# davnords/octic-vits

Measured on AMD Instinct MI355X. Metric: images/sec Hybrid Octic ViT-H/14 224² bf16 train step @1/2/4/8 MI355X, higher is better.
Workload: dtype bf16; 1 GPU; hybrid_deit_huge_patch14 (16 octic + 16 standard blocks, drop_path 0.5) DeiT-III train step: bf16-autocast fwd + bwd + LAMB + EMA, 224x224, batch 64/GPU (BASELINE configs[1]), data parallel over 1 GPU(s); global_batch=64, per_gpu_batch=64, accum_steps=1, parallelism=dp1, library_gemm_table=True, launch=hipGraph replay (whole step)

## Files before the change

include/octic_hip.h:

```cpp
#ifndef OCTIC_HIP_H
#define OCTIC_HIP_H

#include <stdint.h>

#ifdef __cplusplus
extern "C" {
#endif

#define OCTIC_ABI_VERSION 20

enum { OCTIC_F32 = 0, OCTIC_BF16 = 1, OCTIC_U8 = 2  };

enum {
  OCTIC_OK = 0,
  OCTIC_ESHAPE = -1,
  OCTIC_EALIGN = -2,
  OCTIC_EDTYPE = -3,
  OCTIC_ENULL = -4,
  OCTIC_EWORKSPACE = -5
};

typedef struct {
  void* ptr[5];
  int64_t ld[5];
// ... 3 lines not shown
const char* octic_strerror(int code);

enum {
  OCTIC_ROUTE_DENSE_TILE = 0,
  OCTIC_ROUTE_DENSE_SPLIT = 1,
  OCTIC_ROUTE_WGRAD_SLABS = 2,
  OCTIC_ROUTE_WGRAD_TILE = 3,
  OCTIC_ROUTE_LINEAR_RING = 4,
  OCTIC_ROUTE_RING_EVEN = 5,
  OCTIC_ROUTE_ATTN_LEGACY = 6,
  OCTIC_ROUTE_ATTN_ONLINE = 7,
  OCTIC_ROUTE_ATTN_BWD_PAIR = 8,
  OCTIC_ROUTE_DENSE_IMAGE = 9,
  OCTIC_ROUTE_DENSE_CLS2 = 10,
  OCTIC_ROUTE_ATTN_STREAM = 11,
  OCTIC_ROUTE_COUNT = 12
};
int octic_route_override(int knob, int value);

int octic_gelu_d8_fwd(const octic_view* x, const octic_view* y, int64_t M, int c, int dtype, void* stream);
int octic_gelu_d8_bwd(const octic_view* g, const octic_view* x, const octic_view* gin, int64_t M, int c,
                      int dtype, void* stream);
int octic_gelu_d8_fwd_skip(const octic_view* x, const octic_view* y, int64_t M, int c, int dtype,
                           const float* sample_scale, int64_t rows_per_sample, void* stream);
int octic_gelu_d8_bwd_skip(const octic_view* g, const octic_view* x, const octic_view* gin, int64_t M, int c, int dtype,
                           const float* sample_scale, int64_t rows_per_sample, void* stream);

int octic_layernorm_d8_fwd(const octic_view* x, const octic_view* y, const float* const alpha[5],
                           const float* beta, float* stats, int64_t M, int c, float eps, int out_dtype,
                           void* stream);
int octic_layernorm_d8_bwd_blocks(int64_t M);
// ... 66 lines not shown
int octic_linear_d8_ring_order_dropped(int ngroups, const int* items, const int* ksteps, int slots_per_xcd, const int* n_chunks,
                                       const unsigned char* dead_long, const unsigned char* dead_short, int* out_group,
                                       int* out_item, int* out_dead);

int octic_linear_d8_wgrad_has_colsum(int cin, int cout, int dtype);
enum {
  OCTIC_WGRAD_RING = 0,
  OCTIC_WGRAD_TILED = 1
};
int octic_linear_d8_wgrad_plan(int64_t M, int cin, int cout, int dtype, int out[4]);
int64_t octic_linear_d8_wgrad_workspace_bytes(int cin, int cout, int splits);
int octic_linear_d8_wgrad_splits(int64_t M, int cin, int cout);
int octic_linear_d8_wgrad_tile(int64_t M, int cin, int cout);
int octic_linear_d8_wgrad(const octic_view* x, const octic_view* dy, int64_t M, int cin, int cout, int dtype,
                          float* workspace, int splits, void* stream);
int octic_linear_d8_wgrad_finish(const float* workspace, int splits, int cin, int cout,
                                 const float* const w32[5], const float* const cs[5], const float* bias,
                                 const float* dysum, float* const dw[5], float* const dcs[5], float* dbias,
                                 void* stream);
typedef struct octic_wgrad_finish_job {
  const float* workspace;
  const float* w32[5];
  const float* cs[5];
  const float* bias;
  const float* dysum;
  float* dw[5];
  float* dcs[5];
  float* dbias;
  int splits, cin, cout, has_cs;
} octic_wgrad_finish_job;
// ... 406 lines not shown
```

octic_vits_amd/_lib.py:

```python
import ctypes
import os
import re

HERE = os.path.dirname(os.path.abspath(__file__))
LIB_PATH = os.environ.get("OCTIC_LIB") or os.path.join(HERE, "liboctic_hip.so")
HEADER_PATH = os.path.join(HERE, "..", "include", "octic_hip.h")

F32, BF16, U8 = 0, 1, 2
ABI_VERSION = 20
(ROUTE_DENSE_TILE, ROUTE_DENSE_SPLIT, ROUTE_WGRAD_SLABS, ROUTE_WGRAD_TILE, ROUTE_LINEAR_RING, ROUTE_RING_EVEN,
 ROUTE_ATTN_LEGACY, ROUTE_ATTN_ONLINE, ROUTE_ATTN_BWD_PAIR, ROUTE_DENSE_IMAGE, ROUTE_DENSE_CLS2, ROUTE_ATTN_STREAM) = range(12)

DENSE_ADAPT_WIDE, DENSE_ADAPT_NARROW = 16, 32
DENSE_IMAGE_ALWAYS, DENSE_IMAGE_CLS_APART, DENSE_IMAGE_NEVER = 4, 8, 16

(ATTN_FWD_PERSIST, ATTN_FWD_A80_ONESHOT, ATTN_FWD_A80_ONLINE, ATTN_FWD_RESIDENT, ATTN_FWD_STREAM, ATTN_FWD_F32) = range(6)
ATTN_BWD_SINGLE, ATTN_BWD_PAIR, ATTN_BWD_STREAM, ATTN_BWD_F32 = range(4)
LINEAR_WREG, LINEAR_RING, LINEAR_CLASSIC = range(3)
WGRAD_RING, WGRAD_TILED = range(2)
DENSE_F32_NT, DENSE_F32_NN, DENSE_F32_TN = range(3)

c_i64, c_int, c_float, c_void_p = ctypes.c_int64, ctypes.c_int, ctypes.c_float, ctypes.c_void_p
c_double = ctypes.c_double


class OcticView(ctypes.Structure):
# ... 28 lines not shown
    "octic_linear_d8_fwd": (c_int, [VP, c_void_p, c_void_p, VP, VP, c_void_p, c_i64, c_void_p, c_i64, c_int, c_int,
                                    c_int, c_int, c_void_p]),
    "octic_linear_d8_fwd_skip": (c_int, [VP, c_void_p, c_void_p, VP, VP, c_void_p, c_i64, c_void_p, c_i64, c_int, c_int,
                                         c_int, c_int, c_void_p, c_i64, c_void_p]),
    "octic_linear_d8_fwd_dropped": (c_int, [VP, c_void_p, c_void_p, VP, VP, c_void_p, c_i64, c_void_p, c_i64, c_int, c_int,
                                            c_int, c_int, c_void_p, c_i64, c_void_p]),
    "octic_linear_d8_tile_n": (c_int, [c_i64, c_int, c_int]),
    "octic_linear_d8_plan": (c_int, [c_i64, c_int, c_int, c_int, c_int, c_int, ctypes.POINTER(c_int)]),
    "octic_linear_d8_ring_order": (c_int, [c_void_p, c_void_p, c_void_p, c_int, c_void_p, c_void_p]),
    "octic_linear_d8_ring_order_dropped": (c_int, [c_int, c_void_p, c_void_p, c_int, c_void_p, c_void_p, c_void_p, c_void_p,
                                                   c_void_p, c_void_p]),
    "octic_linear_d8_wgrad_tile": (c_int, [c_i64, c_int, c_int]),
    "octic_linear_d8_wgrad_workspace_bytes": (c_i64, [c_int, c_int, c_int]),
    "octic_linear_d8_wgrad_splits": (c_int, [c_i64, c_int, c_int]),
    "octic_linear_d8_wgrad": (c_int, [VP, VP, c_i64, c_int, c_int, c_int, c_void_p, c_int, c_void_p]),
    "octic_linear_d8_wgrad_finish": (c_int, [c_void_p, c_int, c_int, c_int, c_void_p, c_void_p, c_void_p, c_void_p,
                                             c_void_p, c_void_p, c_void_p, c_void_p]),
    "octic_linear_d8_wgrad_finish_batch": (c_int, [c_void_p, c_int, c_void_p]),
    "octic_linear_d8_wgrad_has_colsum": (c_int, [c_int, c_int, c_int]),
    "octic_linear_d8_wgrad_plan": (c_int, [c_i64, c_int, c_int, c_int, ctypes.POINTER(c_int)]),
    "octic_lamb_workspace_floats": (c_i64, [c_int, c_int]),
    "octic_lamb_step": (c_int, [c_void_p] * 10 + [c_int, c_int, c_void_p, c_float, c_float, c_float, c_float, c_float,
                                                  c_int, c_float, c_void_p, c_void_p]),
    "octic_adamw_step": (c_int, [c_void_p] * 10 + [c_int, c_int, c_void_p, c_float, c_float, c_float, c_float, c_float,
                                                   c_int, c_float, c_void_p, c_void_p]),
    "octic_lamb_step_hp": (c_int, [c_void_p] * 10 + [c_int, c_int, c_void_p, c_void_p, c_float, c_float, c_float, c_float,
                                                     c_int, c_void_p, c_void_p, c_void_p]),
    "octic_adamw_step_hp": (c_int, [c_void_p] * 10 + [c_int, c_int, c_void_p, c_void_p, c_float, c_float, c_float, c_float,
                                                      c_int, c_void_p, c_void_p, c_void_p]),
    "octic_dense_blocks": (c_int, [c_i64]),
# ... 214 lines not shown
            raise RuntimeError("octic_vits_amd: ABI version mismatch between _lib.py and liboctic_hip.so")
        _LIB = L
    return _LIB


def route_override(knob: int, value: int) -> int:
    old = lib().octic_route_override(knob, value)
    if old < 0:
        raise ValueError(f"octic_route_override: unknown knob {knob}")
    _PLANS.clear()
    for drop in _ON_OVERRIDE:
        drop()
    return old


_ON_OVERRIDE = []


def on_route_override(drop):
    if drop not in _ON_OVERRIDE:
        _ON_OVERRIDE.append(drop)
    return drop


_PLANS = {}


def plan(query, *args):
    key = (query, args)
    answer = _PLANS.get(key, 0)
# ... 20 lines not shown
```

octic_vits_amd/csrc/elementwise.hip:

```cpp
#include <stdlib.h>
#include "octic_common.hpp"

namespace octic {

template <typename T>
__device__ inline void comp_ptrs(const View& v, int64_t m, int j, int c, T* p[8]) {
#pragma unroll
  for (int i = 0; i < 4; ++i) p[i] = (T*)v.p[i] + m * v.ld[i] + j;
  T* e = (T*)v.p[4] + m * v.ld[4] + j;
  p[4] = e; p[5] = e + 2 * c; p[6] = e + c; p[7] = e + 3 * c;
}

template <typename T, int CH> struct LoadCH;
template <> struct LoadCH<float, 4> {
  static __device__ inline void load(const float* p, float v[4]) { f32x4 a = *(const f32x4*)p; v[0] = a[0]; v[1] = a[1]; v[2] = a[2]; v[3] = a[3]; }
  static __device__ inline void store(float* p, const float v[4]) { *(f32x4*)p = f32x4{v[0], v[1], v[2], v[3]}; }
};
template <> struct LoadCH<bf16, 4> {
  static __device__ inline void load(const bf16* p, float v[4]) { bf16x4 a = *(const bf16x4*)p; v[0] = (float)a[0]; v[1] = (float)a[1]; v[2] = (float)a[2]; v[3] = (float)a[3]; }
  static __device__ inline void store(bf16* p, const float v[4]) { *(bf16x4*)p = bf16x4{(bf16)v[0], (bf16)v[1], (bf16)v[2], (bf16)v[3]}; }
};

struct RowMask {
  const float* ss;
// ... 641 lines not shown
  return OCTIC_OK;
}

template <int SCATTER>
__global__ __launch_bounds__(256) void sample_blocks_kernel(const char* __restrict__ src, char* __restrict__ dst,
                                                            const int64_t* __restrict__ idx, int64_t block_bytes) {
  const int64_t i = blockIdx.y;
  const int64_t j = idx[i];
  const char* s = src + (SCATTER ? i : j) * block_bytes;
  char* d = dst + (SCATTER ? j : i) * block_bytes;
  const int64_t n16 = block_bytes >> 4;
  for (int64_t k = (int64_t)blockIdx.x * 256 + threadIdx.x; k < n16; k += (int64_t)gridDim.x * 256)
    ((u32x4*)d)[k] = ((const u32x4*)s)[k];
}

int g_route[OCTIC_ROUTE_COUNT] = {};

}

using namespace octic;

extern "C" {

int octic_abi_version(void) { return OCTIC_ABI_VERSION; }

int octic_route_override(int knob, int value) {
  if (knob < 0 || knob >= OCTIC_ROUTE_COUNT) return OCTIC_ESHAPE;
  const int old = octic::g_route[knob];
  octic::g_route[knob] = value;
  return old;
}

const char* octic_strerror(int code) {
  switch (code) {
    case OCTIC_OK: return "ok";
    case OCTIC_ESHAPE: return "octic: bad shape (c must be a positive multiple of 8; sizes positive; heads must divide c)";
    case OCTIC_EALIGN: return "octic: pointer or row stride breaks 16-byte row alignment";
    case OCTIC_EDTYPE: return "octic: unsupported dtype combination";
    case OCTIC_ENULL: return "octic: required pointer is NULL";
    case OCTIC_EWORKSPACE: return "octic: workspace too small";
    default: return code > 0 ? hipGetErrorString((hipError_t)code) : "octic: unknown error";
  }
// ... 216 lines not shown
```

octic_vits_amd/csrc/octic_common.hpp:

```cpp
#pragma once
#include <hip/hip_runtime.h>
#include <stdint.h>
#include "../../include/octic_hip.h"

namespace octic {

extern int g_route[OCTIC_ROUTE_COUNT];
inline int route(int knob) { return g_route[knob]; }

typedef __bf16 bf16;
typedef __attribute__((ext_vector_type(8))) __bf16 bf16x8;
typedef __attribute__((ext_vector_type(4))) __bf16 bf16x4;
typedef __attribute__((ext_vector_type(4))) float f32x4;
typedef __attribute__((ext_vector_type(2))) float f32x2;
typedef __attribute__((ext_vector_type(4))) short s16x4;
typedef __attribute__((ext_vector_type(4))) unsigned int u32x4;

constexpr float kSqrt2Over4 = 0.35355339059327376220f;
constexpr float kSqrt1Over2 = 0.70710678118654752440f;
constexpr float kInvSqrt2Pi = 0.39894228040143267794f;

struct View {
  char* p[5];
  int64_t ld[5];
// ... 175 lines not shown
```

octic_vits_amd/csrc/wgrad.hip:

```cpp
#include <stdlib.h>
#include "octic_common.hpp"

namespace octic {

struct WgGroup {
  const char* x;
  int64_t x_ld;
  const char* dy;
  int64_t dy_ld;
  int64_t rows;
  int K, N;
  int pair;
  int k_tiles, n_tiles;
  int wg_begin;
  int splits;
  int64_t slab_off;
  float* colsum;
};
struct WgArgs {
  WgGroup g[5];
  int ngroups;
  int wgs;
  int64_t slab_elems;
  float* slabs;
};

template <typename T> struct WElem;
template <> struct WElem<float> { static constexpr int EPC = 4; static constexpr int BMR = 32; };
template <> struct WElem<bf16> { static constexpr int EPC = 8; static constexpr int BMR = 64; };

template <typename TIN, int TT>
__global__ __launch_bounds__(256) void wgrad_kernel(WgArgs args) {
  constexpr int EPC = WElem<TIN>::EPC;
  constexpr int BMR = WElem<TIN>::BMR;
  constexpr int BW = 32 * TT;
  constexpr int CPR = BW / EPC;
  constexpr int RS = BW * (int)sizeof(TIN) + 16;
  constexpr int TILE = BMR * RS;
  extern __shared__ __attribute__((aligned(16))) char lds[];
// ... 135 lines not shown
#ifndef OCTIC_WG_STAGES
#define OCTIC_WG_STAGES 3
#endif
constexpr int kWgS = OCTIC_WG_STAGES, kWgR = 32;
constexpr int kWgTile = kWgR * 320;
constexpr int kWgStage = 2 * kWgTile;
__device__ __attribute__((aligned(256))) unsigned char g_wg_zero[512];

__device__ inline void wg_wait_tiles(int ahead) {
  if (ahead <= 0) asm volatile("s_waitcnt vmcnt(0)" ::: "memory");
  else if (ahead == 1) asm volatile("s_waitcnt vmcnt(5)" ::: "memory");
  else if (ahead == 2) asm volatile("s_waitcnt vmcnt(10)" ::: "memory");
  else asm volatile("s_waitcnt vmcnt(15)" ::: "memory");
}

__global__ __launch_bounds__(256, 2) void wgrad_ring_kernel(WgArgs args) {
  constexpr int TT = 5, BW = 160;
  extern __shared__ __attribute__((aligned(16))) char lds[];
  const int nwg = gridDim.x, bid = blockIdx.x;
  const int xcd = bid & 7, q8 = nwg >> 3, r8 = nwg & 7;
  const int lid = (xcd < r8 ? xcd * (q8 + 1) : r8 * (q8 + 1) + (xcd - r8) * q8) + (bid >> 3);
  int gi = 0;
#pragma unroll
  for (int i = 1; i < 5; ++i)
    if (i < args.ngroups && lid >= args.g[i].wg_begin) gi = i;
  const WgGroup& G = args.g[gi];
  const int gt = G.k_tiles * G.n_tiles;
  const int rel = lid - G.wg_begin;
  const int split = rel / gt, lt = rel - split * gt;
  const int kt = lt / G.n_tiles, nt = lt - kt * G.n_tiles;
  const int k0 = kt * BW, n0 = nt * BW;
  const int K = G.K, N = G.N;
  int64_t chunk = (G.rows + G.splits - 1) / G.splits;
  chunk = (chunk + kWgR - 1) / kWgR * kWgR;
  const int64_t r0 = (int64_t)split * chunk;
  const int64_t r1 = r0 + chunk < G.rows ? r0 + chunk : G.rows;
  const int nsteps = r0 < r1 ? (int)((r1 - r0 + kWgR - 1) / kWgR) : 0;

  const int tid = threadIdx.x, lane = tid & 63, wid = tid >> 6;
  const int wk = wid & 1, wn = wid >> 1;
  const int fr = lane & 15, kg = lane >> 4;

  const char* src[5];
  int64_t inc[5];
  int row_in_tile[5], cbyte[5], ldst[5];
#pragma unroll
  for (int j = 0; j < 5; ++j) {
    const int q = wid + 4 * j;
    const bool isY = q >= 10;
    const int qq = isY ? q - 10 : q;
    const int o = qq * 1024 + lane * 16;
    const int row = o / 320;
    const int cpos = (o - row * 320) >> 4;
    const int c = ((row & 8) ? cpos + 18 : cpos) % 20;
    const int64_t mm = r0 + row;
    const int64_t ld = isY ? G.dy_ld : G.x_ld;
    const int width = isY ? N : K;
    const int64_t ro = G.pair ? (mm >> 1) * ld + (mm & 1) * (int64_t)width : mm * ld;
    src[j] = (isY ? G.dy : G.x) + (ro + (isY ? n0 : k0)) * 2 + c * 16;
    inc[j] = (G.pair ? 16 : 32) * ld * 2;
    row_in_tile[j] = row;
    cbyte[j] = c * 16;
    ldst[j] = (isY ? kWgTile : 0) + qq * 1024;
  }
  int l_step = 0, l_stage = 0;
  auto issue = [&]() {
    const unsigned st = lds_offset(lds) + l_stage * kWgStage;
    const bool tail = (int64_t)(l_step + 1) * kWgR > r1 - r0;
#pragma unroll
    for (int j = 0; j < 5; ++j) {
      const char* p = src[j];
      if (tail && r0 + (int64_t)l_step * kWgR + row_in_tile[j] >= r1) p = (const char*)g_wg_zero + cbyte[j];
      dma16_to_lds(st + ldst[j], p);
      src[j] += inc[j];
    }
    l_stage = l_stage == kWgS - 1 ? 0 : l_stage + 1;
    ++l_step;
  };

  f32x4 acc[TT][TT];
#pragma unroll
  for (int i = 0; i < TT; ++i)
#pragma unroll
    for (int j = 0; j < TT; ++j) acc[i][j] = f32x4{0, 0, 0, 0};
  const bool do_cs = G.colsum != nullptr && kt == 0 && wk == 0;
  f32x4 accs[TT];
#pragma unroll
  for (int j = 0; j < TT; ++j) accs[j] = f32x4{0, 0, 0, 0};
  const bf16 one = (bf16)1.0f;
// ... 180 lines not shown
    (void)hipGetLastError();
  }
  wgrad_kernel<TIN, TT><<<t, 256, smem, s>>>(a);
  return launch_status();
}

inline int launch_wgrad_ring(WgArgs& a, hipStream_t s) {
  int t = 0;
  for (int i = 0; i < a.ngroups; ++i) {
    a.g[i].k_tiles = a.g[i].K / 160;
    a.g[i].n_tiles = a.g[i].N / 160;
    a.g[i].wg_begin = t;
    t += a.g[i].k_tiles * a.g[i].n_tiles * a.g[i].splits;
  }
  a.wgs = t;
  static DeviceOnce once;
  if (kWgS * kWgStage > 64 * 1024 && once.first()) {
    (void)hipFuncSetAttribute((const void*)wgrad_ring_kernel, hipFuncAttributeMaxDynamicSharedMemorySize, kWgS * kWgStage);
    (void)hipGetLastError();
  }
  wgrad_ring_kernel<<<t, 256, kWgS * kWgStage, s>>>(a);
  return launch_status();
}

#ifndef OCTIC_WG_TARGET
#define OCTIC_WG_TARGET 512.0
#endif
struct WgPlan {
  int kernel;
  int tt;
  int splits;
};
inline WgPlan wgrad_plan(const WgArgs& a, int dtype) {
  WgPlan p = {dtype == OCTIC_BF16 ? OCTIC_WGRAD_RING : OCTIC_WGRAD_TILED, pick_tt(a), 1};
  for (int i = 0; i < a.ngroups; ++i)
    if ((a.g[i].K % 160) || (a.g[i].N % 160)) p.kernel = OCTIC_WGRAD_TILED;
// ... 50 lines not shown
}

int octic_linear_d8_wgrad_has_colsum(int cin, int cout, int dtype) {
  int out[4];
  return octic_linear_d8_wgrad_plan(1, cin, cout, dtype, out) == OCTIC_OK && out[3];
}
int octic_linear_d8_wgrad_tile(int64_t M, int cin, int cout) {
  int out[4];
  return octic_linear_d8_wgrad_plan(M, cin, cout, OCTIC_F32, out) == OCTIC_OK ? out[1] : 0;
}
int octic_linear_d8_wgrad_splits(int64_t M, int cin, int cout) {
  int out[4];
  return octic_linear_d8_wgrad_plan(M, cin, cout, OCTIC_F32, out) == OCTIC_OK ? out[2] : 1;
}

int octic_linear_d8_wgrad(const octic_view* x, const octic_view* dy, int64_t M, int cin, int cout, int dtype,
                          float* workspace, int splits, void* stream) {
  int e;
  if ((e = check_c_dt(cin, dtype)) || (e = check_c_dt(cout, dtype))) return e;
  if ((e = check_view(x, cin, dtype)) || (e = check_view(dy, cout, dtype))) return e;
  if (!workspace) return OCTIC_ENULL;
  if (M <= 0 || splits <= 0) return OCTIC_ESHAPE;
  WgArgs a = {};
  a.slab_elems = linear_slab_elems(cin, cout);
  a.slabs = workspace;
  d8_group_table(a, M, cin, cout);
  for (int gidx = 0; gidx < 5; ++gidx) {
    const int irrep = d8_group_irrep(gidx);
    const bool isE = irrep == 4;
    WgGroup& g = a.g[gidx];
    g.x = (const char*)x->ptr[irrep];
    g.x_ld = x->ld[irrep];
    g.dy = (const char*)dy->ptr[irrep];
    g.dy_ld = dy->ld[irrep];
    g.splits = group_splits(splits, isE);
    g.slab_off = isE ? (int64_t)4 * cin * cout : (int64_t)irrep * cin * cout;
    g.colsum = irrep == 0 ? workspace + colsum_off_elems(cin, cout, splits) : nullptr;
  }
  if (dtype == OCTIC_F32) return launch_wgrad<float>(a, (hipStream_t)stream);
  if (dtype == OCTIC_BF16) return launch_wgrad<bf16>(a, (hipStream_t)stream);
  return OCTIC_EDTYPE;
}

static int fin_args(FinArgs& a, const float* workspace, int splits, int cin, int cout, const float* const w32[5],
                    const float* const cs[5], const float* bias, const float* dysum, float* const dw[5], float* const dcs[5],
                    float* dbias) {
  if (!workspace || !dw) return OCTIC_ENULL;
  if (splits <= 0 || check_c_dt(cin, OCTIC_F32) || check_c_dt(cout, OCTIC_F32)) return OCTIC_ESHAPE;
  if (cs && (!w32 || !dcs)) return OCTIC_ENULL;
  a = FinArgs{};
  a.ngroups = 5;
  a.slab_elems = linear_slab_elems(cin, cout);
  a.slabs = workspace;
  a.bias = bias;
  a.dysum = dysum;
  a.colsum_part = (!dysum && (dbias || (bias && cs))) ? workspace + colsum_off_elems(cin, cout, splits) : nullptr;
// ... 92 lines not shown
```

octic_vits_amd/functional.py:

```python
import os

import torch

from . import ops


class Octic(tuple):

    def __new__(cls, packed: torch.Tensor, c: int):
        self = super().__new__(cls, ops.split_packed(packed, c))
        self.packed, self.c = packed, c
        return self


def as_packed(xs):
    if isinstance(xs, Octic):
        return xs.packed, xs.c
    if len(xs) != 5:
        raise AssertionError("Input should be a 5-tuple")
    c = xs[0].shape[-1]
    if xs[4].shape[-2:] != (2, 2 * c):
        raise ValueError(f"E irrep must be [..., 2, {2 * c}], got {tuple(xs[4].shape)}")
    return torch.cat([xs[0], xs[1], xs[2], xs[3], xs[4].flatten(-2)], dim=-1), c

# ... 195 lines not shown
    ops._require_cuda(x)
    x_in_dtype = x.dtype
    if x.dtype != dtype:
        x = ops.cast_rowscale(_c(x.float()), None, 1, dtype, cin)
    x = _c(x)
    wb, wt = prep.get(w5, cs5, dtype, cin, cout)
    M = x.numel() // (8 * cin)
    y = torch.empty(x.shape[:-1] + (8 * cout,), dtype=out_dtype, device=x.device)
    b32 = None if bias is None else _c(bias.detach().float())
    cs32 = None if cs5 is None else [_c(s.detach().float()) for s in cs5]
    rs32 = None if rs is None else _c(rs.float())
    ctx.lin = (cin, cout, rps, dtype, cs5 is not None, bias is not None, x_in_dtype, wt)
    return x, wb, M, y, b32, cs32, rs32


def _linear_d8_grads(ctx, x, g, w5, cs32, b32, ss_dx, z_dx=None):
    cin, cout, rps, dtype, has_cs, has_bias, x_in_dtype, wt = ctx.lin
    M = x.numel() // (8 * cin)
    gv, xv = ops.pview(g, cout), ops.pview(x, cin)
    dx = None
    if ctx.needs_input_grad[0]:
        dx = torch.empty(x.shape, dtype=dtype, device=x.device)
        ops.linear_fwd(gv, wt, None, ops.pview(dx, cin), M, cout, cin, dtype, dtype, x, sample_scale=ss_dx, skip_rps=rps,
                       dropped=z_dx, dropped_rps=rps)
        if dx.dtype != x_in_dtype:
            dx = dx.to(x_in_dtype)
    dysum = ops.colsum_a1(gv, M, cout, dtype, x) if (has_bias and not ops.wgrad_has_colsum(cin, cout, dtype)) else None
    w32 = [_c(w.detach().float()) for w in w5] if has_cs else None
    f32_masters = all(w.dtype == torch.float32 for w in w5)
    dw, dcs, dbias = ops.linear_wgrad(xv, gv, M, cin, cout, dtype, x, w32=w32, cs5=cs32, bias=b32, dysum=dysum,
                                      want_bias=has_bias, may_defer=f32_masters, wparams=w5 if f32_masters else None)
    if not f32_masters:
        dw = [d.to(w.dtype) for d, w in zip(dw, w5)]
    return dx, dw, dbias, (dcs if has_cs else [None] * 5)


class LinearD8Fn(torch.autograd.Function):

    @staticmethod
    def forward(ctx, x, wA1, wA2, wB1, wB2, wE, bias, resid, rs, sA1, sA2, sB1, sB2, sE, cin, cout, rps, dtype, prep,
                skip_out=None, skip_dx=None, zero_dx=None):
        w5 = (wA1, wA2, wB1, wB2, wE)
        cs5 = None if sA1 is None else (sA1, sA2, sB1, sB2, sE)
        fused = resid is not None
        out_dtype = resid.dtype if fused else dtype
        handed = x
        x, wb, M, y, b32, cs32, rs32 = _linear_d8_fwd_prep(ctx, x, w5, cs5, bias, rs, cin, cout, rps, dtype, out_dtype, prep)
        rv = ops.pview(_c(resid), cout) if fused else None
        plain = not fused and rs32 is None and cs32 is None
        ss_out = linear_skip_scale(skip_out, rps, M) if plain else None
        dropped = ring_skip_scale(rs32, rps, M) if fused else None
        ops.linear_fwd(ops.pview(x, cin), wb, b32, ops.pview(y, cout), M, cin, cout, dtype, out_dtype, x,
                       resid_v=rv, rs=rs32, rps=rps, cs5=cs32, sample_scale=ss_out, skip_rps=rps, dropped=dropped, dropped_rps=rps)
        ss_dx = linear_skip_scale(skip_dx, rps, M)
        z_dx = ring_skip_scale(zero_dx, rps, M) if (plain and ss_dx is None) else None
        row_skip_fill(handed, row_skip_scale(zero_dx, rps, M) if (plain and ss_dx is None) else None, rps, M)
        ctx.save_for_backward(x, rs32, b32, ss_dx, z_dx, *w5, *(cs32 or []))
        ctx.fused = fused
        return y

    @staticmethod
    def backward(ctx, dy):
        cin, cout, rps, dtype, has_cs = ctx.lin[:5]
        x, rs32, b32, ss_dx, z_dx, *rest = ctx.saved_tensors
        w5, cs32 = rest[:5], (rest[5:] if has_cs else None)
        dy = _c(dy)
        if ctx.fused or rs32 is not None or dy.dtype != dtype:
            g = ops.cast_rowscale(_c(dy.float()), rs32, rps, dtype, cout)
        else:
            g = dy
        dx, dw, dbias, dcs = _linear_d8_grads(ctx, x, g, w5, cs32, b32, ss_dx, z_dx)
        return (dx, *dw, dbias, dy if ctx.fused else None, None, *dcs, None, None, None, None, None, None, None, None)


class LinearD8NormFn(torch.autograd.Function):

    @staticmethod
    def forward(ctx, x, wA1, wA2, wB1, wB2, wE, bias, resid, rs, sA1, sA2, sB1, sB2, sE, cin, cout, rps, dtype, prep,
                a1, a2, b1, b2, ae, beta, eps, skip_dx=None):
        w5 = (wA1, wA2, wB1, wB2, wE)
        cs5 = None if sA1 is None else (sA1, sA2, sB1, sB2, sE)
        x, wb, M, y, b32, cs32, rs32 = _linear_d8_fwd_prep(ctx, x, w5, cs5, bias, rs, cin, cout, rps, dtype, resid.dtype, prep)
        ops.linear_fwd(ops.pview(x, cin), wb, b32, ops.pview(y, cout), M, cin, cout, dtype, resid.dtype, x,
                       resid_v=ops.pview(_c(resid), cout), rs=rs32, rps=rps, cs5=cs32, dropped=ring_skip_scale(rs32, rps, M),
                       dropped_rps=rps)
        alpha = None if a1 is None else [_c(t.float()) for t in (a1, a2, b1, b2, ae)]
# ... 19 lines not shown
            gn = _c(dyn)
            ns, nrps = row_skip_get(ctx, M)
            mine = dres is not None and STREAM_GRADS.take(dres)
            if ops.layernorm_bwd_cast_ok(gn, y, cout) and dtype == torch.bfloat16:
                dy, dal_, dbeta, g = ops.layernorm_bwd_cast(gn, y, stats, alpha, dres, cout, rs32, rps,
                                                            want_param_grads=has_affine, sample_scale=ns, rows_per_sample=nrps,
                                                            inplace=mine and ns is not None)
            else:
                dy, dal_, dbeta = ops.layernorm_bwd(gn, y, stats, alpha, dres, cout, want_param_grads=has_affine,
                                                    sample_scale=ns, rows_per_sample=nrps)
            dal = dal_ if dal_ is not None else dal
            STREAM_GRADS.offer(dy)
        dy = _c(dy)
        if g is None:
            g = ops.cast_rowscale(_c(dy.float()), rs32, rps, dtype, cout)
        dx, dw, dbias, dcs = _linear_d8_grads(ctx, x, g, w5, cs32, b32, ss_dx)
        return (dx, *dw, dbias, dy, None, *dcs, None, None, None, None, None, *dal, dbeta if ctx.has_beta else None, None, None)


class PackHeadsFn(torch.autograd.Function):

    @staticmethod
    def forward(ctx, qkv, H, c):
        B, T = qkv.shape[0], qkv.shape[1]
        ctx.meta = (B, T, H, c)
        q, k, v = ops.pack_heads(_c(qkv), B, T, H, c, 3)
        return q, k, v

    @staticmethod
    def backward(ctx, gq, gk, gv):
        B, T, H, c = ctx.meta
# ... 81 lines not shown
    return whole_sample_mask(rs, rps, M, rows_to) if DENSE_NT_SKIP_DROPPED else None


LINEAR_SKIP_DROPPED = _skip_from_env("OCTIC_LINEAR_SKIP")


def linear_skip_scale(rs, rps, M, rows_to=None):
    return whole_sample_mask(rs, rps, M, rows_to) if LINEAR_SKIP_DROPPED else None


RING_SKIP_DROPPED = _skip_from_env("OCTIC_RING_SKIP")


def ring_skip_scale(rs, rps, M):
    return linear_skip_scale(rs, rps, M) if RING_SKIP_DROPPED else None


ROW_SKIP_DROPPED = _skip_from_env("OCTIC_ROW_SKIP")


def row_skip_scale(rs, rps, M, rows_to=None):
    return whole_sample_mask(rs, rps, M, rows_to) if ROW_SKIP_DROPPED else None


class RowSkipSlot:
    __slots__ = ("scale", "rps", "rows", "fills")

    def __init__(self):
        self.scale, self.rps, self.rows, self.fills = None, 0, 0, 0

# ... 830 lines not shown
```

octic_vits_amd/ops.py:

```python
import ctypes
import operator

import torch

from . import _lib
from ._lib import BF16, F32, OcticView, PtrArray5, check, lib

_DT = {torch.float32: F32, torch.bfloat16: BF16}
_DTN = {torch.float32: "f32", torch.bfloat16: "bf16"}


class KernelTimer:

    def __init__(self):
        self.on = False
        self.records = []
        self.overhead_us = 0.0

    def enable(self):
        self.on, self.records = True, []
        pairs = []
        for _ in range(64):
            e0, e1 = torch.cuda.Event(enable_timing=True), torch.cuda.Event(enable_timing=True)
            e0.record()
# ... 369 lines not shown
        nbytes = M * 8 * cin * es + M * 8 * cout * eo * (2 if resid_v is not None else 1) + 8 * cin * cout * es
        fused = int(resid_v is not None or rs is not None or cs5 is not None)
        KERNEL_TIMER.stop(t, linear_kernel_name(cin, cout, dtype, out_dtype, fused, M), nbytes, 24.0 * M * cin * cout)


def linear_kernel_name(cin, cout, dtype, out_dtype, fused, M):
    kernel, _, fused, _ = _lib.plan("octic_linear_d8_plan", M, cin, cout, dt_code(dtype), dt_code(out_dtype), int(fused))
    if kernel == _lib.LINEAR_WREG:
        return f"linear_d8_wreg_kernel<{_DTN[out_dtype]},{fused}>"
    if kernel == _lib.LINEAR_RING:
        return f"linear_d8_ring_kernel<{_DTN[dtype]},{_DTN[out_dtype]},{fused}>"
    return f"linear_d8_kernel<{_DTN[dtype]},{_DTN[out_dtype]}>"


def linear_wgrad(xv, dyv, M, cin, cout, dtype, ref, w32=None, cs5=None, bias=None, dysum=None, want_bias=False,
                 may_defer=True, wparams=None):
    L = lib()
    dev = ref.device
    kernel, tile, splits, _ = _lib.plan("octic_linear_d8_wgrad_plan", M, cin, cout, dt_code(dtype))
    ws = torch.empty(L.octic_linear_d8_wgrad_workspace_bytes(cin, cout, splits) // 4, dtype=torch.float32, device=dev)
    t = KERNEL_TIMER.start()
    check(L.octic_linear_d8_wgrad(ctypes.byref(xv), ctypes.byref(dyv), M, cin, cout, dt_code(dtype), _p(ws), splits,
                                  _stream(ref)))
    if t is not None:
        es = 2 if dtype == torch.bfloat16 else 4
        name = "wgrad_ring_kernel<bf16>" if kernel == _lib.WGRAD_RING else f"wgrad_kernel<{_DTN[dtype]},{tile // 32}>"
        slab = (splits + (splits + 1) // 2) * 4 * cin * cout * 4
        KERNEL_TIMER.stop(t, name, M * 8 * (cin + cout) * es + slab, 24.0 * M * cin * cout)
    shapes = [(cout, cin)] * 4 + [(2 * cout, 2 * cin)]
    dests = [grad_dest(w, sh) for w, sh in zip(wparams, shapes)] if wparams is not None else [None] * 5
    dw = [d if d is not None else torch.empty(sh, dtype=torch.float32, device=dev) for d, sh in zip(dests, shapes)]
    dcs = None
    if cs5 is not None:
        dcs = [torch.empty(cout, dtype=torch.float32, device=dev) for _ in range(4)]
        dcs.append(torch.empty(2 * cout, dtype=torch.float32, device=dev))
    dbias = torch.empty(cout, dtype=torch.float32, device=dev) if want_bias else None
    landed = [w for w, d in zip(wparams, dests) if d is not None] if wparams is not None else []
    if may_defer and DEFERRED_FINISHES.enabled and DEFERRED_FINISHES.slabs_too and _in_backward():
# ... 1561 lines not shown
```

Before: 1293 images/s.

## Skip dropped-sample row tiles in wgrad ring kernel via live-step bitmap

Adds a SKIP variant of the wgrad ring kernel that takes a per-sample scale. It builds an LDS bitmap of row tiles that contain at least one live (non-dropped) sample and walks only those tiles, so no loads or MFMA work are spent on samples removed by drop_path. An optional mode spreads live tiles evenly across splits instead of keeping fixed split ranges. The Python linear backward now passes the drop-path row scale into wgrad by default through an environment knob. The cost is bitmap-building overhead at kernel start, and with the default fixed-split mode the splits can end up unevenly loaded.

```diff
diff --git a/include/octic_hip.h b/include/octic_hip.h
--- a/include/octic_hip.h
+++ b/include/octic_hip.h
@@ -41,7 +41,8 @@
   OCTIC_ROUTE_DENSE_IMAGE = 9,
   OCTIC_ROUTE_DENSE_CLS2 = 10,
   OCTIC_ROUTE_ATTN_STREAM = 11,
-  OCTIC_ROUTE_COUNT = 12
+  OCTIC_ROUTE_COUNT = 12,
+  OCTIC_ROUTE_WGRAD_RING_DEAL = 16
 };
 int octic_route_override(int knob, int value);
 
@@ -138,6 +139,9 @@
 int octic_linear_d8_wgrad_tile(int64_t M, int cin, int cout);
 int octic_linear_d8_wgrad(const octic_view* x, const octic_view* dy, int64_t M, int cin, int cout, int dtype,
                           float* workspace, int splits, void* stream);
+int octic_linear_d8_wgrad_skip(const octic_view* x, const octic_view* dy, int64_t M, int cin, int cout, int dtype,
+                               const float* sample_scale, int rows_per_sample, float* workspace, int splits, void* stream);
+int octic_linear_d8_wgrad_live_range(const unsigned char* dead, int nsteps, int splits, int deal, int* begin, int* steps);
 int octic_linear_d8_wgrad_finish(const float* workspace, int splits, int cin, int cout,
                                  const float* const w32[5], const float* const cs[5], const float* bias,
                                  const float* dysum, float* const dw[5], float* const dcs[5], float* dbias,
diff --git a/octic_vits_amd/_lib.py b/octic_vits_amd/_lib.py
--- a/octic_vits_amd/_lib.py
+++ b/octic_vits_amd/_lib.py
@@ -10,6 +10,8 @@
 ABI_VERSION = 20
 (ROUTE_DENSE_TILE, ROUTE_DENSE_SPLIT, ROUTE_WGRAD_SLABS, ROUTE_WGRAD_TILE, ROUTE_LINEAR_RING, ROUTE_RING_EVEN,
  ROUTE_ATTN_LEGACY, ROUTE_ATTN_ONLINE, ROUTE_ATTN_BWD_PAIR, ROUTE_DENSE_IMAGE, ROUTE_DENSE_CLS2, ROUTE_ATTN_STREAM) = range(12)
+ROUTE_WGRAD_RING_DEAL = 16
+WGRAD_DEAL_OFF, WGRAD_DEAL_FIXED, WGRAD_DEAL_EVEN = range(3)
 
 DENSE_ADAPT_WIDE, DENSE_ADAPT_NARROW = 16, 32
 DENSE_IMAGE_ALWAYS, DENSE_IMAGE_CLS_APART, DENSE_IMAGE_NEVER = 4, 8, 16
@@ -68,6 +70,8 @@
     "octic_linear_d8_wgrad_workspace_bytes": (c_i64, [c_int, c_int, c_int]),
     "octic_linear_d8_wgrad_splits": (c_int, [c_i64, c_int, c_int]),
     "octic_linear_d8_wgrad": (c_int, [VP, VP, c_i64, c_int, c_int, c_int, c_void_p, c_int, c_void_p]),
+    "octic_linear_d8_wgrad_skip": (c_int, [VP, VP, c_i64, c_int, c_int, c_int, c_void_p, c_int, c_void_p, c_int, c_void_p]),
+    "octic_linear_d8_wgrad_live_range": (c_int, [c_void_p, c_int, c_int, c_int, ctypes.POINTER(c_int), ctypes.POINTER(c_int)]),
     "octic_linear_d8_wgrad_finish": (c_int, [c_void_p, c_int, c_int, c_int, c_void_p, c_void_p, c_void_p, c_void_p,
                                              c_void_p, c_void_p, c_void_p, c_void_p]),
     "octic_linear_d8_wgrad_finish_batch": (c_int, [c_void_p, c_int, c_void_p]),
@@ -312,6 +316,10 @@
     return old
 
 
+def wgrad_ring_deal(mode: int) -> int:
+    return lib().octic_route_override(ROUTE_WGRAD_RING_DEAL, int(mode))
+
+
 _ON_OVERRIDE = []
 
 
diff --git a/octic_vits_amd/csrc/elementwise.hip b/octic_vits_amd/csrc/elementwise.hip
--- a/octic_vits_amd/csrc/elementwise.hip
+++ b/octic_vits_amd/csrc/elementwise.hip
@@ -679,7 +679,7 @@
     ((u32x4*)d)[k] = ((const u32x4*)s)[k];
 }
 
-int g_route[OCTIC_ROUTE_COUNT] = {};
+int g_route[OCTIC_ROUTE_SLOTS] = {};
 
 }
 
@@ -690,7 +690,7 @@
 int octic_abi_version(void) { return OCTIC_ABI_VERSION; }
 
 int octic_route_override(int knob, int value) {
-  if (knob < 0 || knob >= OCTIC_ROUTE_COUNT) return OCTIC_ESHAPE;
+  if (knob < 0 || (knob >= OCTIC_ROUTE_COUNT && knob != OCTIC_ROUTE_WGRAD_RING_DEAL)) return OCTIC_ESHAPE;
   const int old = octic::g_route[knob];
   octic::g_route[knob] = value;
   return old;
diff --git a/octic_vits_amd/csrc/octic_common.hpp b/octic_vits_amd/csrc/octic_common.hpp
--- a/octic_vits_amd/csrc/octic_common.hpp
+++ b/octic_vits_amd/csrc/octic_common.hpp
@@ -5,7 +5,8 @@
 
 namespace octic {
 
-extern int g_route[OCTIC_ROUTE_COUNT];
+constexpr int OCTIC_ROUTE_SLOTS = OCTIC_ROUTE_WGRAD_RING_DEAL + 1;
+extern int g_route[OCTIC_ROUTE_SLOTS];
 inline int route(int knob) { return g_route[knob]; }
 
 typedef __bf16 bf16;
diff --git a/octic_vits_amd/csrc/wgrad.hip b/octic_vits_amd/csrc/wgrad.hip
--- a/octic_vits_amd/csrc/wgrad.hip
+++ b/octic_vits_amd/csrc/wgrad.hip
@@ -23,6 +23,9 @@
   int wgs;
   int64_t slab_elems;
   float* slabs;
+  const float* sample_scale;
+  int rows_per_sample;
+  int deal;
 };
 
 template <typename T> struct WElem;
@@ -188,6 +191,70 @@
   else asm volatile("s_waitcnt vmcnt(15)" ::: "memory");
 }
 
+constexpr int kWgMaskWords = 64;
+struct WgRange {
+  int first;
+  int count;
+};
+template <typename W>
+__host__ __device__ inline WgRange wg_live_range(W word, int nsteps, int S, int s, int deal) {
+  if (deal != 2) {
+    const int q = (nsteps + S - 1) / S;
+    const int a = s * q < nsteps ? s * q : nsteps;
+    const int b = a + q < nsteps ? a + q : nsteps;
+    if (deal == 0) return {a, b - a};
+    int n = 0;
+    for (int w = a >> 6; w < (b + 63) >> 6; ++w) {
+      unsigned long long m = word(w);
+      const int lo = w << 6;
+      if (a > lo) m &= ~0ull << (a - lo);
+      if (b < lo + 64) m &= ~(~0ull << (b - lo));
+      n += __builtin_popcountll(m);
+    }
+    return {a, n};
+  }
+  const int nw = (nsteps + 63) >> 6;
+  int L = 0;
+  for (int w = 0; w < nw; ++w) L += __builtin_popcountll(word(w));
+  const int qL = (L + S - 1) / S;
+  const int lo = s * qL < L ? s * qL : L;
+  const int hi = lo + qL < L ? lo + qL : L;
+  if (lo == hi) return {nsteps, 0};
+  int rank = lo, w = 0;
+  unsigned long long m = word(0);
+  for (int c = __builtin_popcountll(m); rank >= c; c = __builtin_popcountll(m)) {
+    rank -= c;
+    m = word(++w);
+  }
+  int pos = 0;
+#pragma unroll
+  for (int half = 32; half; half >>= 1) {
+    const int c = __builtin_popcountll((m >> pos) & ((1ull << half) - 1));
+    if (rank >= c) {
+      rank -= c;
+      pos += half;
+    }
+  }
+  return {(w << 6) + pos, hi - lo};
+}
+struct WgWalk {
+  int w;
+  unsigned long long m;
+  template <typename W>
+  __host__ __device__ inline void start(W word, int first) {
+    w = first >> 6;
+    m = word(w) & (~0ull << (first & 63));
+  }
+  template <typename W>
+  __host__ __device__ inline int next(W word) {
+    while (m == 0) m = word(++w);
+    const int step = (w << 6) + __builtin_ctzll(m);
+    m &= m - 1;
+    return step;
+  }
+};
+
+template <bool SKIP>
 __global__ __launch_bounds__(256, 2) void wgrad_ring_kernel(WgArgs args) {
   constexpr int TT = 5, BW = 160;
   extern __shared__ __attribute__((aligned(16))) char lds[];
@@ -209,11 +276,34 @@
   chunk = (chunk + kWgR - 1) / kWgR * kWgR;
   const int64_t r0 = (int64_t)split * chunk;
   const int64_t r1 = r0 + chunk < G.rows ? r0 + chunk : G.rows;
-  const int nsteps = r0 < r1 ? (int)((r1 - r0 + kWgR - 1) / kWgR) : 0;
+  int nsteps = r0 < r1 ? (int)((r1 - r0 + kWgR - 1) / kWgR) : 0;
 
   const int tid = threadIdx.x, lane = tid & 63, wid = tid >> 6;
   const int wk = wid & 1, wn = wid >> 1;
   const int fr = lane & 15, kg = lane >> 4;
+
+  __shared__ unsigned long long live_bm[SKIP ? kWgMaskWords : 1];
+  const int gsteps = (int)((G.rows + kWgR - 1) / kWgR);
+  if constexpr (SKIP) {
+    const int wid0 = __builtin_amdgcn_readfirstlane(wid);
+    const WgRange own = wg_live_range([](int) { return 0ull; }, gsteps, G.splits, split, 0);
+    const int w_lo = args.deal == 2 ? 0 : own.first >> 6;
+    const int w_hi = args.deal == 2 ? (gsteps + 63) >> 6 : (own.first + own.count + 63) >> 6;
+    const float* scale = args.sample_scale;
+    const unsigned rps = (unsigned)args.rows_per_sample, rows = (unsigned)G.rows;
+    for (int w = w_lo + wid0; w < w_hi; w += 4) {
+      const unsigned st = (unsigned)(w << 6) + lane;
+      bool live = false;
+      if (st < (unsigned)gsteps) {
+        const unsigned ra = st * kWgR, rb = ra + kWgR - 1 < rows ? ra + kWgR - 1 : rows - 1;
+        const unsigned b1 = (rb >> G.pair) / rps;
+        for (unsigned b = (ra >> G.pair) / rps; b <= b1; ++b) live = live || scale[b] != 0.0f;
+      }
+      const unsigned long long m = __ballot(live);
+      if (lane == 0) live_bm[w] = m;
+    }
+  }
+  const int64_t row_base = SKIP ? 0 : r0;
 
   const char* src[5];
   int64_t inc[5];
@@ -227,7 +317,7 @@
     const int row = o / 320;
     const int cpos = (o - row * 320) >> 4;
     const int c = ((row & 8) ? cpos + 18 : cpos) % 20;
-    const int64_t mm = r0 + row;
+    const int64_t mm = row_base + row;
     const int64_t ld = isY ? G.dy_ld : G.x_ld;
     const int width = isY ? N : K;
     const int64_t ro = G.pair ? (mm >> 1) * ld + (mm & 1) * (int64_t)width : mm * ld;
@@ -237,16 +327,43 @@
     cbyte[j] = c * 16;
     ldst[j] = (isY ? kWgTile : 0) + qq * 1024;
   }
+  auto bm_word = [&](int i) {
+    const unsigned long long v = live_bm[i];
+    return ((unsigned long long)(unsigned)__builtin_amdgcn_readfirstlane((int)(v >> 32)) << 32) |
+           (unsigned)__builtin_amdgcn_readfirstlane((int)v);
+  };
+  WgWalk walk = {0, 0};
+  int g_rows = (int)G.rows;
+  if constexpr (SKIP) {
+    asm volatile("" : "+s"(g_rows));
+    __syncthreads();
+    const WgRange rg = wg_live_range(bm_word, gsteps, G.splits, split, args.deal);
+    nsteps = __builtin_amdgcn_readfirstlane(rg.count);
+    if (nsteps > 0) walk.start(bm_word, __builtin_amdgcn_readfirstlane(rg.first));
+  }
+
   int l_step = 0, l_stage = 0;
   auto issue = [&]() {
     const unsigned st = lds_offset(lds) + l_stage * kWgStage;
-    const bool tail = (int64_t)(l_step + 1) * kWgR > r1 - r0;
-#pragma unroll
-    for (int j = 0; j < 5; ++j) {
-      const char* p = src[j];
-      if (tail && r0 + (int64_t)l_step * kWgR + row_in_tile[j] >= r1) p = (const char*)g_wg_zero + cbyte[j];
-      dma16_to_lds(st + ldst[j], p);
-      src[j] += inc[j];
+    if constexpr (SKIP) {
+      const int step = walk.next(bm_word);
+      const int rb = step * kWgR;
+      const bool tail = rb + kWgR > g_rows;
+#pragma unroll
+      for (int j = 0; j < 5; ++j) {
+        const char* p = src[j] + step * inc[j];
+        if (tail && rb + row_in_tile[j] >= g_rows) p = (const char*)g_wg_zero + cbyte[j];
+        dma16_to_lds(st + ldst[j], p);
+      }
+    } else {
+      const bool tail = (int64_t)(l_step + 1) * kWgR > r1 - r0;
+#pragma unroll
+      for (int j = 0; j < 5; ++j) {
+        const char* p = src[j];
+        if (tail && r0 + (int64_t)l_step * kWgR + row_in_tile[j] >= r1) p = (const char*)g_wg_zero + cbyte[j];
+        dma16_to_lds(st + ldst[j], p);
+        src[j] += inc[j];
+      }
     }
     l_stage = l_stage == kWgS - 1 ? 0 : l_stage + 1;
     ++l_step;
@@ -457,12 +574,18 @@
     t += a.g[i].k_tiles * a.g[i].n_tiles * a.g[i].splits;
   }
   a.wgs = t;
+  a.deal = a.sample_scale ? route(OCTIC_ROUTE_WGRAD_RING_DEAL) : 0;
+  if (a.deal != 1 && a.deal != 2) a.deal = 0;
+  for (int i = 0; i < a.ngroups; ++i)
+    if ((a.g[i].rows + kWgR - 1) / kWgR > kWgMaskWords * 64) a.deal = 0;
   static DeviceOnce once;
   if (kWgS * kWgStage > 64 * 1024 && once.first()) {
-    (void)hipFuncSetAttribute((const void*)wgrad_ring_kernel, hipFuncAttributeMaxDynamicSharedMemorySize, kWgS * kWgStage);
+    (void)hipFuncSetAttribute((const void*)wgrad_ring_kernel<false>, hipFuncAttributeMaxDynamicSharedMemorySize, kWgS * kWgStage);
+    (void)hipFuncSetAttribute((const void*)wgrad_ring_kernel<true>, hipFuncAttributeMaxDynamicSharedMemorySize, kWgS * kWgStage);
     (void)hipGetLastError();
   }
-  wgrad_ring_kernel<<<t, 256, kWgS * kWgStage, s>>>(a);
+  if (a.deal) wgrad_ring_kernel<true><<<t, 256, kWgS * kWgStage, s>>>(a);
+  else wgrad_ring_kernel<false><<<t, 256, kWgS * kWgStage, s>>>(a);
   return launch_status();
 }
 
@@ -543,16 +666,38 @@
   return octic_linear_d8_wgrad_plan(M, cin, cout, OCTIC_F32, out) == OCTIC_OK ? out[2] : 1;
 }
 
-int octic_linear_d8_wgrad(const octic_view* x, const octic_view* dy, int64_t M, int cin, int cout, int dtype,
-                          float* workspace, int splits, void* stream) {
+int octic_linear_d8_wgrad_live_range(const unsigned char* dead, int nsteps, int splits, int deal, int* begin, int* steps) {
+  if (!begin || !steps || (deal && !dead)) return OCTIC_ENULL;
+  if (nsteps <= 0 || nsteps > kWgMaskWords * 64 || splits <= 0 || deal < 0 || deal > 2) return OCTIC_ESHAPE;
+  unsigned long long bm[kWgMaskWords] = {};
+  for (int i = 0; i < nsteps; ++i)
+    if (!deal || !dead[i]) bm[i >> 6] |= 1ull << (i & 63);
+  auto word = [&](int i) { return bm[i]; };
+  int n = 0;
+  for (int s = 0; s < splits; ++s) {
+    begin[s] = n;
+    const WgRange rg = wg_live_range(word, nsteps, splits, s, deal);
+    WgWalk walk = {0, 0};
+    if (rg.count > 0) walk.start(word, rg.first);
+    for (int i = 0; i < rg.count; ++i) steps[n++] = walk.next(word);
+  }
+  begin[splits] = n;
+  return OCTIC_OK;
+}
+
+int octic_linear_d8_wgrad_skip(const octic_view* x, const octic_view* dy, int64_t M, int cin, int cout, int dtype,
+                               const float* sample_scale, int rows_per_sample, float* workspace, int splits, void* stream) {
   int e;
   if ((e = check_c_dt(cin, dtype)) || (e = check_c_dt(cout, dtype))) return e;
   if ((e = check_view(x, cin, dtype)) || (e = check_view(dy, cout, dtype))) return e;
   if (!workspace) return OCTIC_ENULL;
   if (M <= 0 || splits <= 0) return OCTIC_ESHAPE;
+  if (sample_scale && (rows_per_sample <= 0 || M % rows_per_sample != 0)) return OCTIC_ESHAPE;
   WgArgs a = {};
   a.slab_elems = linear_slab_elems(cin, cout);
   a.slabs = workspace;
+  a.sample_scale = sample_scale;
+  a.rows_per_sample = rows_per_sample;
   d8_group_table(a, M, cin, cout);
   for (int gidx = 0; gidx < 5; ++gidx) {
     const int irrep = d8_group_irrep(gidx);
@@ -569,6 +714,11 @@
   if (dtype == OCTIC_F32) return launch_wgrad<float>(a, (hipStream_t)stream);
   if (dtype == OCTIC_BF16) return launch_wgrad<bf16>(a, (hipStream_t)stream);
   return OCTIC_EDTYPE;
+}
+
+int octic_linear_d8_wgrad(const octic_view* x, const octic_view* dy, int64_t M, int cin, int cout, int dtype,
+                          float* workspace, int splits, void* stream) {
+  return octic_linear_d8_wgrad_skip(x, dy, M, cin, cout, dtype, nullptr, 0, workspace, splits, stream);
 }
 
 static int fin_args(FinArgs& a, const float* workspace, int splits, int cin, int cout, const float* const w32[5],
diff --git a/octic_vits_amd/functional.py b/octic_vits_amd/functional.py
--- a/octic_vits_amd/functional.py
+++ b/octic_vits_amd/functional.py
@@ -2,7 +2,7 @@
 
 import torch
 
-from . import ops
+from . import _lib, ops
 
 
 class Octic(tuple):
@@ -233,7 +233,7 @@
     return x, wb, M, y, b32, cs32, rs32
 
 
-def _linear_d8_grads(ctx, x, g, w5, cs32, b32, ss_dx, z_dx=None):
+def _linear_d8_grads(ctx, x, g, w5, cs32, b32, ss_dx, z_dx=None, z_w=None):
     cin, cout, rps, dtype, has_cs, has_bias, x_in_dtype, wt = ctx.lin
     M = x.numel() // (8 * cin)
     gv, xv = ops.pview(g, cout), ops.pview(x, cin)
@@ -247,8 +247,11 @@
     dysum = ops.colsum_a1(gv, M, cout, dtype, x) if (has_bias and not ops.wgrad_has_colsum(cin, cout, dtype)) else None
     w32 = [_c(w.detach().float()) for w in w5] if has_cs else None
     f32_masters = all(w.dtype == torch.float32 for w in w5)
+    if z_w is not None:
+        _lib.wgrad_ring_deal(WGRAD_RING_SKIP)
     dw, dcs, dbias = ops.linear_wgrad(xv, gv, M, cin, cout, dtype, x, w32=w32, cs5=cs32, bias=b32, dysum=dysum,
-                                      want_bias=has_bias, may_defer=f32_masters, wparams=w5 if f32_masters else None)
+                                      want_bias=has_bias, may_defer=f32_masters, wparams=w5 if f32_masters else None,
+                                      sample_scale=z_w, rows_per_sample=rps)
     if not f32_masters:
         dw = [d.to(w.dtype) for d, w in zip(dw, w5)]
     return dx, dw, dbias, (dcs if has_cs else [None] * 5)
@@ -274,21 +277,22 @@
         ss_dx = linear_skip_scale(skip_dx, rps, M)
         z_dx = ring_skip_scale(zero_dx, rps, M) if (plain and ss_dx is None) else None
         row_skip_fill(handed, row_skip_scale(zero_dx, rps, M) if (plain and ss_dx is None) else None, rps, M)
-        ctx.save_for_backward(x, rs32, b32, ss_dx, z_dx, *w5, *(cs32 or []))
+        z_w = wgrad_ring_skip_scale(rs32 if rs32 is not None else (zero_dx if plain else None), rps, M)
+        ctx.save_for_backward(x, rs32, b32, ss_dx, z_dx, z_w, *w5, *(cs32 or []))
         ctx.fused = fused
         return y
 
     @staticmethod
     def backward(ctx, dy):
         cin, cout, rps, dtype, has_cs = ctx.lin[:5]
-        x, rs32, b32, ss_dx, z_dx, *rest = ctx.saved_tensors
+        x, rs32, b32, ss_dx, z_dx, z_w, *rest = ctx.saved_tensors
         w5, cs32 = rest[:5], (rest[5:] if has_cs else None)
         dy = _c(dy)
         if ctx.fused or rs32 is not None or dy.dtype != dtype:
             g = ops.cast_rowscale(_c(dy.float()), rs32, rps, dtype, cout)
         else:
             g = dy
-        dx, dw, dbias, dcs = _linear_d8_grads(ctx, x, g, w5, cs32, b32, ss_dx, z_dx)
+        dx, dw, dbias, dcs = _linear_d8_grads(ctx, x, g, w5, cs32, b32, ss_dx, z_dx, z_w)
         return (dx, *dw, dbias, dy if ctx.fused else None, None, *dcs, None, None, None, None, None, None, None, None)
 
 
@@ -338,7 +342,7 @@
         dy = _c(dy)
         if g is None:
             g = ops.cast_rowscale(_c(dy.float()), rs32, rps, dtype, cout)
-        dx, dw, dbias, dcs = _linear_d8_grads(ctx, x, g, w5, cs32, b32, ss_dx)
+        dx, dw, dbias, dcs = _linear_d8_grads(ctx, x, g, w5, cs32, b32, ss_dx, z_w=wgrad_ring_skip_scale(rs32, rps, M))
         return (dx, *dw, dbias, dy, None, *dcs, None, None, None, None, None, *dal, dbeta if ctx.has_beta else None, None, None)
 
 
@@ -450,6 +454,16 @@
 
 def ring_skip_scale(rs, rps, M):
     return linear_skip_scale(rs, rps, M) if RING_SKIP_DROPPED else None
+
+
+WGRAD_RING_SKIP_DEFAULT = 1
+WGRAD_RING_SKIP = int(os.environ.get("OCTIC_WGRAD_RING_SKIP", str(WGRAD_RING_SKIP_DEFAULT)).strip() or 0)
+if WGRAD_RING_SKIP not in (0, 1, 2):
+    raise ValueError("OCTIC_WGRAD_RING_SKIP must be 0 (off), 1 (fixed splits) or 2 (dealt evenly)")
+
+
+def wgrad_ring_skip_scale(rs, rps, M):
+    return linear_skip_scale(rs, rps, M) if WGRAD_RING_SKIP else None
 
 
 ROW_SKIP_DROPPED = _skip_from_env("OCTIC_ROW_SKIP")
diff --git a/octic_vits_amd/ops.py b/octic_vits_amd/ops.py
--- a/octic_vits_amd/ops.py
+++ b/octic_vits_amd/ops.py
@@ -407,14 +407,15 @@
 
 
 def linear_wgrad(xv, dyv, M, cin, cout, dtype, ref, w32=None, cs5=None, bias=None, dysum=None, want_bias=False,
-                 may_defer=True, wparams=None):
+                 may_defer=True, wparams=None, sample_scale=None, rows_per_sample=0):
     L = lib()
     dev = ref.device
+    ss, srps = _sample_scale(sample_scale, rows_per_sample, M, ref, "linear_wgrad")
     kernel, tile, splits, _ = _lib.plan("octic_linear_d8_wgrad_plan", M, cin, cout, dt_code(dtype))
     ws = torch.empty(L.octic_linear_d8_wgrad_workspace_bytes(cin, cout, splits) // 4, dtype=torch.float32, device=dev)
     t = KERNEL_TIMER.start()
-    check(L.octic_linear_d8_wgrad(ctypes.byref(xv), ctypes.byref(dyv), M, cin, cout, dt_code(dtype), _p(ws), splits,
-                                  _stream(ref)))
+    check(L.octic_linear_d8_wgrad_skip(ctypes.byref(xv), ctypes.byref(dyv), M, cin, cout, dt_code(dtype), _p(ss), srps, _p(ws),
+                                       splits, _stream(ref)))
     if t is not None:
         es = 2 if dtype == torch.bfloat16 else 4
         name = "wgrad_ring_kernel<bf16>" if kernel == _lib.WGRAD_RING else f"wgrad_kernel<{_DTN[dtype]},{tile // 32}>"
```

Result: no change. 1304 images/s, median of 6 (+0.9%).
